# megapose6d/megapose6d

Hardware: NVIDIA H100
Metric: pose hypotheses/sec through render+coarse+5x refine (higher is better)
Workload: dtype f16

## Files before the change

megapose6d_b200/csrc/conv_wgmma.cu:

```cuda
#include <cuda.h>
#include <vector>
#include "mpx_common.cuh"

namespace mpx {

#ifdef MPX_ACT_BF16
#define kTmaActType CU_TENSOR_MAP_DATA_TYPE_BFLOAT16
#define MPX_WGMMA_AB "bf16.bf16"
#else
#define kTmaActType CU_TENSOR_MAP_DATA_TYPE_FLOAT16
#define MPX_WGMMA_AB "f16.f16"
#endif

__device__ __forceinline__ void mbar_init(uint64_t* bar, uint32_t count) {
  asm volatile("mbarrier.init.shared::cta.b64 [%0], %1;" ::"r"(smem_u32(bar)), "r"(count));
}
__device__ __forceinline__ void mbar_expect_tx(uint64_t* bar, uint32_t bytes) {
  asm volatile("mbarrier.arrive.expect_tx.shared::cta.b64 _, [%0], %1;" ::"r"(smem_u32(bar)), "r"(bytes) : "memory");
}
__device__ __forceinline__ void mbar_arrive(uint64_t* bar) {
  asm volatile("mbarrier.arrive.shared::cta.b64 _, [%0];" ::"r"(smem_u32(bar)) : "memory");
}
__device__ __forceinline__ bool mbar_try_wait(uint64_t* bar, uint32_t parity) {
  uint32_t ok;
// ... 34 lines not shown
__device__ __forceinline__ void wgmma_commit() { asm volatile("wgmma.commit_group.sync.aligned;" ::: "memory"); }
template <int N>
__device__ __forceinline__ void wgmma_wait() {
  asm volatile("wgmma.wait_group.sync.aligned %0;" ::"n"(N) : "memory");
}

__device__ __forceinline__ void wgmma_m64n64k16(float (&d)[32], uint64_t desc_a, uint64_t desc_b, uint32_t accumulate) {
  asm volatile(
      "{\n\t.reg .pred p;\n\tsetp.ne.b32 p, %34, 0;\n\t"
      "wgmma.mma_async.sync.aligned.m64n64k16.f32." MPX_WGMMA_AB " "
      "{%0, %1, %2, %3, %4, %5, %6, %7, %8, %9, %10, %11, %12, %13, %14, %15, %16, %17, %18, %19, %20, %21, %22, %23, %24, %25, %26, %27, %28, %29, %30, %31}, %32, %33, p, 1, 1, 0, 0;\n\t}"
      : "+f"(d[0]), "+f"(d[1]), "+f"(d[2]), "+f"(d[3]), "+f"(d[4]), "+f"(d[5]), "+f"(d[6]), "+f"(d[7]), "+f"(d[8]), "+f"(d[9]), "+f"(d[10]), "+f"(d[11]), "+f"(d[12]), "+f"(d[13]), "+f"(d[14]), "+f"(d[15]), "+f"(d[16]), "+f"(d[17]), "+f"(d[18]), "+f"(d[19]), "+f"(d[20]), "+f"(d[21]), "+f"(d[22]), "+f"(d[23]), "+f"(d[24]), "+f"(d[25]), "+f"(d[26]), "+f"(d[27]), "+f"(d[28]), "+f"(d[29]), "+f"(d[30]), "+f"(d[31])
      : "l"(desc_a), "l"(desc_b), "r"(accumulate)
      : "memory");
}
__device__ __forceinline__ void wgmma_m64n128k16(float (&d)[64], uint64_t desc_a, uint64_t desc_b, uint32_t accumulate) {
  asm volatile(
      "{\n\t.reg .pred p;\n\tsetp.ne.b32 p, %66, 0;\n\t"
      "wgmma.mma_async.sync.aligned.m64n128k16.f32." MPX_WGMMA_AB " "
      "{%0, %1, %2, %3, %4, %5, %6, %7, %8, %9, %10, %11, %12, %13, %14, %15, %16, %17, %18, %19, %20, %21, %22, %23, %24, %25, %26, %27, %28, %29, %30, %31, %32, %33, %34, %35, %36, %37, %38, %39, %40, %41, %42, %43, %44, %45, %46, %47, %48, %49, %50, %51, %52, %53, %54, %55, %56, %57, %58, %59, %60, %61, %62, %63}, %64, %65, p, 1, 1, 0, 0;\n\t}"
      : "+f"(d[0]), "+f"(d[1]), "+f"(d[2]), "+f"(d[3]), "+f"(d[4]), "+f"(d[5]), "+f"(d[6]), "+f"(d[7]), "+f"(d[8]), "+f"(d[9]), "+f"(d[10]), "+f"(d[11]), "+f"(d[12]), "+f"(d[13]), "+f"(d[14]), "+f"(d[15]), "+f"(d[16]), "+f"(d[17]), "+f"(d[18]), "+f"(d[19]), "+f"(d[20]), "+f"(d[21]), "+f"(d[22]), "+f"(d[23]), "+f"(d[24]), "+f"(d[25]), "+f"(d[26]), "+f"(d[27]), "+f"(d[28]), "+f"(d[29]), "+f"(d[30]), "+f"(d[31]), "+f"(d[32]), "+f"(d[33]), "+f"(d[34]), "+f"(d[35]), "+f"(d[36]), "+f"(d[37]), "+f"(d[38]), "+f"(d[39]), "+f"(d[40]), "+f"(d[41]), "+f"(d[42]), "+f"(d[43]), "+f"(d[44]), "+f"(d[45]), "+f"(d[46]), "+f"(d[47]), "+f"(d[48]), "+f"(d[49]), "+f"(d[50]), "+f"(d[51]), "+f"(d[52]), "+f"(d[53]), "+f"(d[54]), "+f"(d[55]), "+f"(d[56]), "+f"(d[57]), "+f"(d[58]), "+f"(d[59]), "+f"(d[60]), "+f"(d[61]), "+f"(d[62]), "+f"(d[63])
      : "l"(desc_a), "l"(desc_b), "r"(accumulate)
      : "memory");
}
__device__ __forceinline__ void wgmma_m64n256k16(float (&d)[128], uint64_t desc_a, uint64_t desc_b, uint32_t accumulate) {
  asm volatile(
      "{\n\t.reg .pred p;\n\tsetp.ne.b32 p, %130, 0;\n\t"
      "wgmma.mma_async.sync.aligned.m64n256k16.f32." MPX_WGMMA_AB " "
      "{%0, %1, %2, %3, %4, %5, %6, %7, %8, %9, %10, %11, %12, %13, %14, %15, %16, %17, %18, %19, %20, %21, %22, %23, %24, %25, %26, %27, %28, %29, %30, %31, %32, %33, %34, %35, %36, %37, %38, %39, %40, %41, %42, %43, %44, %45, %46, %47, %48, %49, %50, %51, %52, %53, %54, %55, %56, %57, %58, %59, %60, %61, %62, %63, %64, %65, %66, %67, %68, %69, %70, %71, %72, %73, %74, %75, %76, %77, %78, %79, %80, %81, %82, %83, %84, %85, %86, %87, %88, %89, %90, %91, %92, %93, %94, %95, %96, %97, %98, %99, %100, %101, %102, %103, %104, %105, %106, %107, %108, %109, %110, %111, %112, %113, %114, %115, %116, %117, %118, %119, %120, %121, %122, %123, %124, %125, %126, %127}, %128, %129, p, 1, 1, 0, 0;\n\t}"
      : "+f"(d[0]), "+f"(d[1]), "+f"(d[2]), "+f"(d[3]), "+f"(d[4]), "+f"(d[5]), "+f"(d[6]), "+f"(d[7]), "+f"(d[8]), "+f"(d[9]), "+f"(d[10]), "+f"(d[11]), "+f"(d[12]), "+f"(d[13]), "+f"(d[14]), "+f"(d[15]), "+f"(d[16]), "+f"(d[17]), "+f"(d[18]), "+f"(d[19]), "+f"(d[20]), "+f"(d[21]), "+f"(d[22]), "+f"(d[23]), "+f"(d[24]), "+f"(d[25]), "+f"(d[26]), "+f"(d[27]), "+f"(d[28]), "+f"(d[29]), "+f"(d[30]), "+f"(d[31]), "+f"(d[32]), "+f"(d[33]), "+f"(d[34]), "+f"(d[35]), "+f"(d[36]), "+f"(d[37]), "+f"(d[38]), "+f"(d[39]), "+f"(d[40]), "+f"(d[41]), "+f"(d[42]), "+f"(d[43]), "+f"(d[44]), "+f"(d[45]), "+f"(d[46]), "+f"(d[47]), "+f"(d[48]), "+f"(d[49]), "+f"(d[50]), "+f"(d[51]), "+f"(d[52]), "+f"(d[53]), "+f"(d[54]), "+f"(d[55]), "+f"(d[56]), "+f"(d[57]), "+f"(d[58]), "+f"(d[59]), "+f"(d[60]), "+f"(d[61]), "+f"(d[62]), "+f"(d[63]), "+f"(d[64]), "+f"(d[65]), "+f"(d[66]), "+f"(d[67]), "+f"(d[68]), "+f"(d[69]), "+f"(d[70]), "+f"(d[71]), "+f"(d[72]), "+f"(d[73]), "+f"(d[74]), "+f"(d[75]), "+f"(d[76]), "+f"(d[77]), "+f"(d[78]), "+f"(d[79]), "+f"(d[80]), "+f"(d[81]), "+f"(d[82]), "+f"(d[83]), "+f"(d[84]), "+f"(d[85]), "+f"(d[86]), "+f"(d[87]), "+f"(d[88]), "+f"(d[89]), "+f"(d[90]), "+f"(d[91]), "+f"(d[92]), "+f"(d[93]), "+f"(d[94]), "+f"(d[95]), "+f"(d[96]), "+f"(d[97]), "+f"(d[98]), "+f"(d[99]), "+f"(d[100]), "+f"(d[101]), "+f"(d[102]), "+f"(d[103]), "+f"(d[104]), "+f"(d[105]), "+f"(d[106]), "+f"(d[107]), "+f"(d[108]), "+f"(d[109]), "+f"(d[110]), "+f"(d[111]), "+f"(d[112]), "+f"(d[113]), "+f"(d[114]), "+f"(d[115]), "+f"(d[116]), "+f"(d[117]), "+f"(d[118]), "+f"(d[119]), "+f"(d[120]), "+f"(d[121]), "+f"(d[122]), "+f"(d[123]), "+f"(d[124]), "+f"(d[125]), "+f"(d[126]), "+f"(d[127])
      : "l"(desc_a), "l"(desc_b), "r"(accumulate)
      : "memory");
}
template <int BLOCK_N>
__device__ __forceinline__ void wgmma_tile(float (&d)[BLOCK_N / 2], uint64_t da, uint64_t db, uint32_t accumulate) {
  if constexpr (BLOCK_N == 64) wgmma_m64n64k16(d, da, db, accumulate);
  else if constexpr (BLOCK_N == 128) wgmma_m64n128k16(d, da, db, accumulate);
  else wgmma_m64n256k16(d, da, db, accumulate);
}

__device__ __forceinline__ uint64_t make_sw128_desc(uint32_t smem_addr) {
  uint64_t d = 0;
  d |= static_cast<uint64_t>((smem_addr >> 4) & 0x3FFFu);
  d |= static_cast<uint64_t>(1) << 16;
  d |= static_cast<uint64_t>(64) << 32;
  d |= static_cast<uint64_t>(1) << 62;
  return d;
}

__device__ __forceinline__ uint32_t cluster_ctarank() {
  uint32_t r;
  asm volatile("mov.u32 %0, %%cluster_ctarank;" : "=r"(r));
  return r;
}
__device__ __forceinline__ void cluster_sync_all() {
  asm volatile("barrier.cluster.arrive.release.aligned;" ::: "memory");
  asm volatile("barrier.cluster.wait.acquire.aligned;" ::: "memory");
}
__device__ __forceinline__ void consumers_sync() { asm volatile("bar.sync 1, 256;" ::: "memory"); }

__device__ __forceinline__ void red_max_act4(act_t* dst, uint32_t lo, uint32_t hi) {
#ifdef MPX_ACT_BF16
  asm volatile("red.global.max.noftz.v2.bf16x2 [%0], {%1, %2};" ::"l"(dst), "r"(lo), "r"(hi) : "memory");
#else
  asm volatile("red.global.max.noftz.v2.f16x2 [%0], {%1, %2};" ::"l"(dst), "r"(lo), "r"(hi) : "memory");
#endif
}

struct ProfileSlot {
  cudaEvent_t e0, e1;
// ... 302 lines not shown
        const int px0 = x >> 1, px1 = ((x & 1) && ((x + 1) >> 1) < pq2) ? (x + 1) >> 1 : px0;
        for (int py = py0; py <= py1; ++py) {
          for (int px = px0; px <= px1; ++px) {
            act_t* dst = p.out + ((static_cast<size_t>(img) * pp + py) * pq2 + px) * p.C_out + n0 + col;
#pragma unroll
            for (int j = 0; j < BLOCK_N / 8; ++j) red_max_act4(dst + 8 * j, packed[j], nb[j]);
          }
        }
      }
    }
  }

  __syncthreads();
  if (p.splits > 1) {
    cluster_sync_all();
    const int item = blockIdx.x;
    const int tile = item / p.splits;
    const int m_tile = tile / p.n_tiles;
    const int n_tile = tile - m_tile * p.n_tiles;
    const int n0 = n_tile * BLOCK_N;
    splitk_reduce_slice<BLOCK_N>(smem_u32(smem), p.splits, static_cast<int>(cluster_ctarank()),
                                 static_cast<long long>(m_tile) * kBlockM, p.M_total, p.C_out, n0, p.out, p.residual,
                                 bias_s + n0, p.relu, threadIdx.x, blockDim.x);
    cluster_sync_all();
  }
}

constexpr int kC64Pixels = 256;
constexpr int kC64Stages = 4;
constexpr int kC64ActBytes = kC64Pixels * kBlockK * 2;
constexpr int kC64WBytes = 64 * kBlockK * 2;
constexpr int kC64StageBytes = kC64ActBytes + kC64WBytes;
constexpr int kC64StagingBytes = kC64Pixels * 64 * 2;
constexpr int kC64SmemBytes = kC64Stages * kC64StageBytes + 2 * kC64StagingBytes + 1024  +
                              128  + 256 ;
static_assert(kC64SmemBytes <= 227 * 1024, "conv64: shared memory budget");

struct Conv64Params {
  int M_total, P, Q, S, stride, pad_h, pad_w, cblocks, num_k_blocks, m_tiles;
  int relu;
  int has_residual;
  const float* bias;
};

__device__ __forceinline__ void tma_store_2d(const CUtensorMap* map, const void* smem, int c0, int c1) {
  asm volatile("cp.async.bulk.tensor.2d.global.shared::cta.bulk_group [%0, {%2, %3}], [%1];" ::"l"(map),
               "r"(smem_u32(smem)), "r"(c0), "r"(c1)
               : "memory");
}
__device__ __forceinline__ void bulk_commit() { asm volatile("cp.async.bulk.commit_group;" ::: "memory"); }
__device__ __forceinline__ void bulk_wait_read_all() { asm volatile("cp.async.bulk.wait_group.read 0;" ::: "memory"); }
__device__ __forceinline__ void bulk_wait_all() { asm volatile("cp.async.bulk.wait_group 0;" ::: "memory"); }
__device__ __forceinline__ void fence_proxy_async_smem() { asm volatile("fence.proxy.async.shared::cta;" ::: "memory"); }
__device__ __forceinline__ void warpgroup_sync(int cw) { asm volatile("bar.sync %0, 128;" ::"r"(2 + cw) : "memory"); }
__device__ __forceinline__ void mainloop_turn_wait(int cw) { asm volatile("bar.sync %0, 256;" ::"r"(4 + cw) : "memory"); }
__device__ __forceinline__ void mainloop_turn_pass(int cw) { asm volatile("bar.arrive %0, 256;" ::"r"(5 - cw) : "memory"); }

__host__ __device__ __forceinline__ uint32_t stem_live_steps(int kb, int cblocks, int S) {
  const int tap = kb / cblocks, cb = kb - tap * cblocks;
  const int r = tap / S, s = tap - r * S;
  uint32_t live = 0;
  for (int k = 0; k < 4; ++k) {
    const int slice = (4 * cb + k) / cblocks;
    const int ky = 2 * r + (slice >> 1) - 1, kx = 2 * s + (slice & 1) - 1;
    if (ky >= 0 && ky <= 6 && kx >= 0 && kx <= 6) live |= 1u << k;
  }
  return live;
}

__device__ __forceinline__ void wgmma_kblock(uint32_t live, float (&acc)[128], uint64_t da, uint64_t db) {
  wgmma_fence();
#pragma unroll
  for (int k = 0; k < kBlockK / 16; ++k)
    if (live & (1u << k)) wgmma_m64n256k16(acc, da + static_cast<uint64_t>(2 * k), db + static_cast<uint64_t>(2 * k), 1u);
  wgmma_commit();
}

template <int kStemCblocks>
__global__ void __launch_bounds__(kThreads, 1)
conv64_wgmma_kernel(const __grid_constant__ CUtensorMap map_x, const __grid_constant__ CUtensorMap map_w,
                    const __grid_constant__ CUtensorMap map_res, const __grid_constant__ CUtensorMap map_out,
                    const Conv64Params p) {
  extern __shared__ uint8_t smem_raw[];
  uint8_t* smem = reinterpret_cast<uint8_t*>((reinterpret_cast<uintptr_t>(smem_raw) + 1023) &
                                             ~static_cast<uintptr_t>(1023));
  uint8_t* smem_x = smem;
  uint8_t* smem_w = smem + kC64Stages * kC64ActBytes;
  uint8_t* staging = smem + kC64Stages * kC64StageBytes;
  uint64_t* bars = reinterpret_cast<uint64_t*>(staging + 2 * kC64StagingBytes);
  uint64_t* full_bar = bars;
  uint64_t* empty_bar = bars + kC64Stages;
  uint64_t* res_bar = bars + 2 * kC64Stages;
  float* bias_s = reinterpret_cast<float*>(bars + 16);

  const int wg = __shfl_sync(0xffffffffu, threadIdx.x >> 7, 0);
  const int nk = p.num_k_blocks;
  for (int i = threadIdx.x; i < 64; i += blockDim.x) bias_s[i] = p.bias[i];
  if (threadIdx.x == 0) {
    asm volatile("prefetch.tensormap [%0];" ::"l"(&map_x) : "memory");
    asm volatile("prefetch.tensormap [%0];" ::"l"(&map_w) : "memory");
    asm volatile("prefetch.tensormap [%0];" ::"l"(&map_out) : "memory");
    if (p.has_residual) asm volatile("prefetch.tensormap [%0];" ::"l"(&map_res) : "memory");
    for (int i = 0; i < kC64Stages; ++i) {
      mbar_init(&full_bar[i], 1);
      mbar_init(&empty_bar[i], 4);
    }
    mbar_init(&res_bar[0], 1);
    mbar_init(&res_bar[1], 1);
    asm volatile("fence.mbarrier_init.release.cluster;" ::: "memory");
  }
  pdl_trigger();
  __syncthreads();
  pdl_wait();

  if (wg == 0) {
    asm volatile("setmaxnreg.dec.sync.aligned.u32 40;");
    if (threadIdx.x == 0) {
      int stage = 0;
      uint32_t phase = 0;
      const int pq = p.P * p.Q;
      for (int tile = blockIdx.x; tile < p.m_tiles; tile += gridDim.x) {
        int base_w[2], base_h[2], img[2];
        const int m0 = tile * kC64Pixels;
        const bool second = m0 + kBlockM < p.M_total;
#pragma unroll
        for (int hh = 0; hh < 2; ++hh) {
          const int m = m0 + hh * kBlockM;
          img[hh] = m / pq;
          const int rem = m - img[hh] * pq;
          const int p0 = rem / p.Q;
          base_w[hh] = (rem - p0 * p.Q) * p.stride - p.pad_w;
          base_h[hh] = p0 * p.stride - p.pad_h;
        }
        const uint32_t bytes = (second ? kC64ActBytes : kC64ActBytes / 2) + kC64WBytes;
        int tap = 0, cb = 0;
        for (int kb = 0; kb < nk; ++kb) {
          mbar_wait(&empty_bar[stage], phase ^ 1u);
          mbar_expect_tx(&full_bar[stage], bytes);
          const int r = tap / p.S;
          const int s = tap - r * p.S;
          uint8_t* dst = smem_x + stage * kC64ActBytes;
          tma_load_im2col_4d(dst, &map_x, &full_bar[stage], cb * kBlockK, base_w[0], base_h[0], img[0],
                             static_cast<uint16_t>(s), static_cast<uint16_t>(r));
          if (second)
            tma_load_im2col_4d(dst + kATileBytes, &map_x, &full_bar[stage], cb * kBlockK, base_w[1], base_h[1], img[1],
                               static_cast<uint16_t>(s), static_cast<uint16_t>(r));
          tma_load_2d(smem_w + stage * kC64WBytes, &map_w, &full_bar[stage], kb * kBlockK, 0);
          if (++cb == p.cblocks) {
            cb = 0;
            ++tap;
          }
          if (++stage == kC64Stages) {
            stage = 0;
            phase ^= 1u;
          }
        }
      }
    }
  } else {
    asm volatile("setmaxnreg.inc.sync.aligned.u32 232;");
    const int cw = wg - 1;
    const int t = threadIdx.x & 127;
    const int lane = threadIdx.x & 31;
    const int q = lane >> 2;
    const int c = 16 * (t >> 5) + (q & ~1);
    const int px = 2 * (lane & 3) + (q & 1);
    const bool odd = (q & 1) != 0;
    uint8_t* stage_buf = staging + cw * kC64StagingBytes;
    int local = 0;
    for (int i = cw, tile = blockIdx.x + cw * gridDim.x; tile < p.m_tiles; i += 2, tile += 2 * gridDim.x, ++local) {
      const int m0 = tile * kC64Pixels;
      if (p.has_residual && t == 0) {
        bulk_wait_read_all();
        mbar_expect_tx(&res_bar[cw], kC64StagingBytes);
        tma_load_2d(stage_buf, &map_res, &res_bar[cw], 0, m0);
      }
      const uint32_t g = static_cast<uint32_t>(i) * static_cast<uint32_t>(nk);
      int stage = static_cast<int>(g % kC64Stages);
      uint32_t phase = (g / kC64Stages) & 1u;
      float acc[128];
#pragma unroll
      for (int j = 0; j < 128; ++j) acc[j] = 0.f;
      if (i > 0) mainloop_turn_wait(cw);
      int prev_stage = -1;
      auto kblock = [&](uint32_t live) {
        mbar_wait(&full_bar[stage], phase);
        wgmma_kblock(live, acc, make_sw128_desc(smem_u32(smem_w + stage * kC64WBytes)),
                     make_sw128_desc(smem_u32(smem_x + stage * kC64ActBytes)));
        wgmma_wait<1>();
        if (prev_stage >= 0) {
          __syncwarp();
          if (lane == 0) mbar_arrive(&empty_bar[prev_stage]);
        }
        prev_stage = stage;
        if (++stage == kC64Stages) {
          stage = 0;
          phase ^= 1u;
        }
      };
      if constexpr (kStemCblocks > 0) {
#pragma unroll
        for (int kb = 0; kb < 16 * kStemCblocks; ++kb) kblock(stem_live_steps(kb, kStemCblocks, 4));
      } else {
#pragma unroll 1
        for (int kb = 0; kb < nk; ++kb) kblock(0xFu);
      }
      if (tile + static_cast<int>(gridDim.x) < p.m_tiles) mainloop_turn_pass(cw);
      wgmma_wait<0>();
      __syncwarp();
      if (lane == 0) mbar_arrive(&empty_bar[prev_stage]);

      if (t == 0) bulk_wait_read_all();
      warpgroup_sync(cw);
      if (p.has_residual) mbar_wait(&res_bar[cw], static_cast<uint32_t>(local) & 1u);
      const uint32_t sbase = smem_u32(stage_buf);
#pragma unroll
      for (int h = 0; h < 2; ++h) {
        const float2 b = *reinterpret_cast<const float2*>(bias_s + c + 8 * h);
        const int chunk = (c + 8 * h) >> 3;
#pragma unroll
        for (int j = 0; j < 32; ++j) {
          const float v0 = acc[4 * j + 2 * h], v1 = acc[4 * j + 2 * h + 1];
          const float other = __shfl_xor_sync(0xffffffffu, odd ? v0 : v1, 4);
          float f0 = (odd ? other : v0) + b.x;
          float f1 = (odd ? v1 : other) + b.y;
          const int row = 8 * j + px;
          const uint32_t addr =
              sbase + static_cast<uint32_t>(row * 128 + ((chunk ^ px) << 4) + ((c & 7) << 1));
          if (p.has_residual) {
            uint32_t rr;
            asm volatile("ld.shared.b32 %0, [%1];" : "=r"(rr) : "r"(addr) : "memory");
            const float2 r = unpack_act2(rr);
            f0 += r.x;
            f1 += r.y;
          }
          if (p.relu) {
            f0 = fmaxf(f0, 0.f);
            f1 = fmaxf(f1, 0.f);
          }
          asm volatile("st.shared.b32 [%0], %1;" ::"r"(addr), "r"(pack_act2(f0, f1)) : "memory");
        }
      }
      fence_proxy_async_smem();
      warpgroup_sync(cw);
      if (t == 0) {
        tma_store_2d(&map_out, stage_buf, 0, m0);
        bulk_commit();
      }
    }
    if (t == 0) bulk_wait_all();
  }
}

typedef CUresult (*PFN_encodeTiled)(CUtensorMap*, CUtensorMapDataType, cuuint32_t, void*,
                                    const cuuint64_t*, const cuuint64_t*, const cuuint32_t*,
                                    const cuuint32_t*, CUtensorMapInterleave, CUtensorMapSwizzle,
                                    CUtensorMapL2promotion, CUtensorMapFloatOOBfill);
typedef CUresult (*PFN_encodeIm2col)(CUtensorMap*, CUtensorMapDataType, cuuint32_t, void*,
                                     const cuuint64_t*, const cuuint64_t*, const int*, const int*,
                                     cuuint32_t, cuuint32_t, const cuuint32_t*, CUtensorMapInterleave,
                                     CUtensorMapSwizzle, CUtensorMapL2promotion,
                                     CUtensorMapFloatOOBfill);

static PFN_encodeTiled g_encode_tiled = nullptr;
static PFN_encodeIm2col g_encode_im2col = nullptr;

static int load_driver_entry_points() {
  if (g_encode_tiled && g_encode_im2col) return MPX_OK;
  cudaDriverEntryPointQueryResult q;
  void* f = nullptr;
  MPX_CHECK_CUDA(cudaGetDriverEntryPoint("cuTensorMapEncodeTiled", &f, cudaEnableDefault, &q));
  MPX_REQUIRE(f != nullptr && q == cudaDriverEntryPointSuccess,
              "cuTensorMapEncodeTiled not available from the driver");
  g_encode_tiled = reinterpret_cast<PFN_encodeTiled>(f);
  f = nullptr;
  MPX_CHECK_CUDA(cudaGetDriverEntryPoint("cuTensorMapEncodeIm2col", &f, cudaEnableDefault, &q));
  MPX_REQUIRE(f != nullptr && q == cudaDriverEntryPointSuccess,
              "cuTensorMapEncodeIm2col not available from the driver");
  g_encode_im2col = reinterpret_cast<PFN_encodeIm2col>(f);
// ... 33 lines not shown
                           static_cast<cuuint64_t>(d.W) * d.C_in * 2,
                           static_cast<cuuint64_t>(d.H) * d.W * d.C_in * 2};
  int lower[2] = {-d.pad_lo_w, -d.pad_lo_h};
  int upper[2] = {d.pad_hi_w - (d.S - 1), d.pad_hi_h - (d.R - 1)};
  cuuint32_t estr[4] = {1, static_cast<cuuint32_t>(d.stride), static_cast<cuuint32_t>(d.stride), 1};
  CUresult r = g_encode_im2col(map, kTmaActType, 4, const_cast<void*>(x),
                               dims, strides, lower, upper, kBlockK,
                               kBlockM, estr, CU_TENSOR_MAP_INTERLEAVE_NONE,
                               CU_TENSOR_MAP_SWIZZLE_128B, CU_TENSOR_MAP_L2_PROMOTION_L2_128B,
                               CU_TENSOR_MAP_FLOAT_OOB_FILL_NONE);
  MPX_REQUIRE(r == CUDA_SUCCESS, "cuTensorMapEncodeIm2col failed (%d)", static_cast<int>(r));
  int drv = 0;
  cudaDriverGetVersion(&drv);
  const size_t bytes = static_cast<size_t>(d.n_img) * d.H * d.W * d.C_in * 2;
  if (drv <= 13010 && bytes < 131072) {
    reinterpret_cast<uint64_t*>(map)[1] &= ~(1ull << 21);
  }
  return MPX_OK;
}

static int encode_2d_map(CUtensorMap* map, const void* ptr, cuuint64_t cols, cuuint64_t rows, int box_cols, int box_rows,
                         CUtensorMapL2promotion promo) {
  cuuint64_t dims[2] = {cols, rows};
  cuuint64_t strides[1] = {cols * 2};
  cuuint32_t box[2] = {static_cast<cuuint32_t>(box_cols), static_cast<cuuint32_t>(box_rows)};
  cuuint32_t estr[2] = {1, 1};
  CUresult r = g_encode_tiled(map, kTmaActType, 2, const_cast<void*>(ptr), dims, strides, box, estr,
                              CU_TENSOR_MAP_INTERLEAVE_NONE, CU_TENSOR_MAP_SWIZZLE_128B, promo,
                              CU_TENSOR_MAP_FLOAT_OOB_FILL_NONE);
  MPX_REQUIRE(r == CUDA_SUCCESS, "cuTensorMapEncodeTiled failed (%d)", static_cast<int>(r));
  return MPX_OK;
}

static int conv64_forward(const ConvDesc& d, const CUtensorMap& map_x, const void* w, const float* bias,
                          const void* residual, void* out, int M_total, int P, int Q, int cap, cudaStream_t stream) {
  const int K_total = d.R * d.S * d.C_in;
  CUtensorMap map_w, map_res, map_out;
  int rc = encode_2d_map(&map_w, w, K_total, 64, kBlockK, 64, CU_TENSOR_MAP_L2_PROMOTION_L2_256B);
  if (rc != MPX_OK) return rc;
  rc = encode_2d_map(&map_out, out, 64, M_total, 64, kC64Pixels, CU_TENSOR_MAP_L2_PROMOTION_L2_128B);
  if (rc != MPX_OK) return rc;
  map_res = map_out;
  if (residual != nullptr) {
    rc = encode_2d_map(&map_res, residual, 64, M_total, 64, kC64Pixels, CU_TENSOR_MAP_L2_PROMOTION_L2_128B);
    if (rc != MPX_OK) return rc;
  }
  Conv64Params p{};
  p.M_total = M_total;
  p.P = P;
  p.Q = Q;
  p.S = d.S;
  p.stride = d.stride;
  p.pad_h = d.pad_lo_h;
  p.pad_w = d.pad_lo_w;
  p.cblocks = d.C_in / kBlockK;
  p.num_k_blocks = d.R * d.S * p.cblocks;
  p.m_tiles = (M_total + kC64Pixels - 1) / kC64Pixels;
  p.relu = d.relu;
  p.has_residual = residual != nullptr;
  p.bias = bias;
  const int stem_cblocks = (d.s2d_stem && d.R == 4 && d.S == 4 && p.cblocks <= 2) ? p.cblocks : 0;
  long long live_steps = 0;
  for (int kb = 0; kb < p.num_k_blocks; ++kb)
    live_steps += __builtin_popcount(stem_cblocks ? stem_live_steps(kb, p.cblocks, p.S) : 0xFu);

  static bool attr_set = false;
  if (!attr_set) {
    MPX_CHECK_CUDA(cudaFuncSetAttribute(conv64_wgmma_kernel<0>, cudaFuncAttributeMaxDynamicSharedMemorySize,
                                        kC64SmemBytes));
    MPX_CHECK_CUDA(cudaFuncSetAttribute(conv64_wgmma_kernel<1>, cudaFuncAttributeMaxDynamicSharedMemorySize,
                                        kC64SmemBytes));
    MPX_CHECK_CUDA(cudaFuncSetAttribute(conv64_wgmma_kernel<2>, cudaFuncAttributeMaxDynamicSharedMemorySize,
                                        kC64SmemBytes));
    attr_set = true;
  }
  const int grid = p.m_tiles < cap ? p.m_tiles : cap;
  ProfileSlot* slot = profile_begin(stream);
  void (*kernel)(CUtensorMap, CUtensorMap, CUtensorMap, CUtensorMap, Conv64Params) =
      stem_cblocks == 1 ? conv64_wgmma_kernel<1> : (stem_cblocks == 2 ? conv64_wgmma_kernel<2> : conv64_wgmma_kernel<0>);
  MPX_CHECK_CUDA(launch_pdl(kernel, dim3(grid), dim3(kThreads), kC64SmemBytes, stream, 1, map_x, map_w, map_res, map_out,
                            p));
  MPX_CHECK_CUDA(cudaGetLastError());
  ++g_launches;
  profile_end(slot, stream, 2.0 * M_total * 64 * live_steps * 16);
  return MPX_OK;
}

int conv_forward(const ConvDesc& d, const void* x, const void* w, const float* bias,
                 const void* residual, void* out, int block_n_override, int max_ctas,
                 cudaStream_t stream, int splitk) {
  MPX_REQUIRE(d.C_in % 64 == 0 && d.C_in >= 64, "conv: C_in=%d must be a multiple of 64", d.C_in);
  MPX_REQUIRE(d.C_out % 64 == 0 && d.C_out <= 512, "conv: C_out=%d must be a multiple of 64, at most 512", d.C_out);
  MPX_REQUIRE(d.stride == 1 || d.stride == 2, "conv: stride %d unsupported", d.stride);
  MPX_REQUIRE(d.R >= 1 && d.R <= 8 && d.S >= 1 && d.S <= 8, "conv: filter %dx%d unsupported", d.R, d.S);
  if (d.pool && (!d.relu || residual != nullptr || block_n_override != 0 || splitk != 0)) return MPX_ERR_UNSUPPORTED;
  int rc = load_driver_entry_points();
  if (rc != MPX_OK) return rc;

  const int P = conv_out_dim(d.H, d.pad_lo_h, d.pad_hi_h, d.R, d.stride);
  const int Q = conv_out_dim(d.W, d.pad_lo_w, d.pad_hi_w, d.S, d.stride);
  MPX_REQUIRE(P > 0 && Q > 0, "conv: empty output");
  const long long M_total = static_cast<long long>(d.n_img) * P * Q;
  MPX_REQUIRE(M_total > 0 && M_total < (1LL << 31), "conv: M=%lld out of range", M_total);

  int block_n = block_n_override;
  if (block_n <= 0) {
    const long long m_tiles_est = (M_total + kBlockM - 1) / kBlockM;
    block_n = d.C_out % 256 == 0 ? 256 : (d.C_out % 128 == 0 ? 128 : 64);
    while (block_n > 64 && m_tiles_est * (d.C_out / block_n) < 32) block_n /= 2;
  }
  MPX_REQUIRE((block_n == 64 || block_n == 128 || block_n == 256) && d.C_out % block_n == 0,
              "conv: BLOCK_N=%d invalid for C_out=%d", block_n, d.C_out);

  CUtensorMap map_a, map_b;
  rc = encode_im2col_map(&map_a, d, x);
  if (rc != MPX_OK) return rc;

  const bool aligned = (reinterpret_cast<uintptr_t>(out) & 15) == 0 && (reinterpret_cast<uintptr_t>(residual) & 15) == 0;
  const long long tiles256 = (M_total + kC64Pixels - 1) / kC64Pixels;
  const int cap = max_ctas > 0 ? max_ctas : sm_count();
  if (d.C_out == 64 && block_n_override == 0 && splitk <= 0 && !d.pool && aligned && (g_conv_mode & 4194304) == 0 &&
      ((g_conv_mode & 67108864) != 0 || tiles256 >= 2LL * cap)) {
    const long long m_tiles128 = (M_total + kBlockM - 1) / kBlockM;
    const int nkb = d.R * d.S * (d.C_in / kBlockK);
    if (!(splitk < 0 && m_tiles128 * 2 <= cap && nkb >= 8))
      return conv64_forward(d, map_a, w, bias, residual, out, static_cast<int>(M_total), P, Q, cap, stream);
  }

  rc = encode_2d_map(&map_b, w, static_cast<cuuint64_t>(d.R) * d.S * d.C_in, d.C_out, kBlockK, block_n,
                     CU_TENSOR_MAP_L2_PROMOTION_L2_256B);
  if (rc != MPX_OK) return rc;

  ConvParams p{};
  p.M_total = static_cast<int>(M_total);
  p.P = P;
  p.Q = Q;
  p.C_out = d.C_out;
  p.S = d.S;
  p.stride = d.stride;
  p.pad_h = d.pad_lo_h;
  p.pad_w = d.pad_lo_w;
  p.cblocks = d.C_in / kBlockK;
  p.num_k_blocks = d.R * d.S * p.cblocks;
  p.m_tiles = static_cast<int>((M_total + kBlockM - 1) / kBlockM);
  p.n_tiles = d.C_out / block_n;
  p.relu = d.relu;
  p.pool = d.pool;
  p.bias = bias;
  p.residual = reinterpret_cast<const act_t*>(residual);
  p.out = reinterpret_cast<act_t*>(out);
  p.splits = 1;
  if (splitk != 0) {
    const int tiles = p.m_tiles * p.n_tiles;
    const int sms = max_ctas > 0 ? max_ctas : sm_count();
    int want = splitk > 0 ? splitk : 1;
    if (splitk < 0 && tiles * 2 <= sms && p.num_k_blocks >= 8) {
      want = p.num_k_blocks / 4;
      if (want > sms / tiles) want = sms / tiles;
    }
    const int cap = (splitk < 0 && (g_conv_mode & 524288)) ? 1 : ((splitk < 0 && (g_conv_mode & 262144)) ? 2 : 8);
    int splits = 1;
// ... 16 lines not shown
```

Before: 21560.

## Add row-band producer with resident weights to C_out=64 conv kernel

For stride-1 convs whose padded width fits in a 256-pixel tile, the conv64 kernel now loads a band of input rows once per (row tap, channel block) with a plain 4D tiled TMA. It reuses that band across the S horizontal taps by offsetting the smem descriptor, instead of issuing one im2col load per tap. When they fit, all weights are kept resident in shared memory for the whole kernel. An N=160 wgmma variant handles narrower bands. This cuts redundant activation traffic and weight reloads, at the cost of wasted MMA columns on padded pixels and a more complex barrier scheme.

```diff
diff --git a/megapose6d_b200/csrc/conv_wgmma.cu b/megapose6d_b200/csrc/conv_wgmma.cu
--- a/megapose6d_b200/csrc/conv_wgmma.cu
+++ b/megapose6d_b200/csrc/conv_wgmma.cu
@@ -90,10 +90,20 @@
       : "l"(desc_a), "l"(desc_b), "r"(accumulate)
       : "memory");
 }
+__device__ __forceinline__ void wgmma_m64n160k16(float (&d)[80], uint64_t desc_a, uint64_t desc_b, uint32_t accumulate) {
+  asm volatile(
+      "{\n\t.reg .pred p;\n\tsetp.ne.b32 p, %82, 0;\n\t"
+      "wgmma.mma_async.sync.aligned.m64n160k16.f32." MPX_WGMMA_AB " "
+      "{%0, %1, %2, %3, %4, %5, %6, %7, %8, %9, %10, %11, %12, %13, %14, %15, %16, %17, %18, %19, %20, %21, %22, %23, %24, %25, %26, %27, %28, %29, %30, %31, %32, %33, %34, %35, %36, %37, %38, %39, %40, %41, %42, %43, %44, %45, %46, %47, %48, %49, %50, %51, %52, %53, %54, %55, %56, %57, %58, %59, %60, %61, %62, %63, %64, %65, %66, %67, %68, %69, %70, %71, %72, %73, %74, %75, %76, %77, %78, %79}, %80, %81, p, 1, 1, 0, 0;\n\t}"
+      : "+f"(d[0]), "+f"(d[1]), "+f"(d[2]), "+f"(d[3]), "+f"(d[4]), "+f"(d[5]), "+f"(d[6]), "+f"(d[7]), "+f"(d[8]), "+f"(d[9]), "+f"(d[10]), "+f"(d[11]), "+f"(d[12]), "+f"(d[13]), "+f"(d[14]), "+f"(d[15]), "+f"(d[16]), "+f"(d[17]), "+f"(d[18]), "+f"(d[19]), "+f"(d[20]), "+f"(d[21]), "+f"(d[22]), "+f"(d[23]), "+f"(d[24]), "+f"(d[25]), "+f"(d[26]), "+f"(d[27]), "+f"(d[28]), "+f"(d[29]), "+f"(d[30]), "+f"(d[31]), "+f"(d[32]), "+f"(d[33]), "+f"(d[34]), "+f"(d[35]), "+f"(d[36]), "+f"(d[37]), "+f"(d[38]), "+f"(d[39]), "+f"(d[40]), "+f"(d[41]), "+f"(d[42]), "+f"(d[43]), "+f"(d[44]), "+f"(d[45]), "+f"(d[46]), "+f"(d[47]), "+f"(d[48]), "+f"(d[49]), "+f"(d[50]), "+f"(d[51]), "+f"(d[52]), "+f"(d[53]), "+f"(d[54]), "+f"(d[55]), "+f"(d[56]), "+f"(d[57]), "+f"(d[58]), "+f"(d[59]), "+f"(d[60]), "+f"(d[61]), "+f"(d[62]), "+f"(d[63]), "+f"(d[64]), "+f"(d[65]), "+f"(d[66]), "+f"(d[67]), "+f"(d[68]), "+f"(d[69]), "+f"(d[70]), "+f"(d[71]), "+f"(d[72]), "+f"(d[73]), "+f"(d[74]), "+f"(d[75]), "+f"(d[76]), "+f"(d[77]), "+f"(d[78]), "+f"(d[79])
+      : "l"(desc_a), "l"(desc_b), "r"(accumulate)
+      : "memory");
+}
 template <int BLOCK_N>
 __device__ __forceinline__ void wgmma_tile(float (&d)[BLOCK_N / 2], uint64_t da, uint64_t db, uint32_t accumulate) {
   if constexpr (BLOCK_N == 64) wgmma_m64n64k16(d, da, db, accumulate);
   else if constexpr (BLOCK_N == 128) wgmma_m64n128k16(d, da, db, accumulate);
+  else if constexpr (BLOCK_N == 160) wgmma_m64n160k16(d, da, db, accumulate);
   else wgmma_m64n256k16(d, da, db, accumulate);
 }
 
@@ -462,12 +472,18 @@
 constexpr int kC64WBytes = 64 * kBlockK * 2;
 constexpr int kC64StageBytes = kC64ActBytes + kC64WBytes;
 constexpr int kC64StagingBytes = kC64Pixels * 64 * 2;
-constexpr int kC64SmemBytes = kC64Stages * kC64StageBytes + 2 * kC64StagingBytes + 1024  +
-                              128  + 256 ;
-static_assert(kC64SmemBytes <= 227 * 1024, "conv64: shared memory budget");
+constexpr int kC64BandSlots = 3;
+constexpr int kC64BandWStages = 8;
+static_assert(kC64BandSlots * kC64ActBytes + kC64BandWStages * kC64WBytes == kC64Stages * kC64StageBytes,
+              "conv64: the band producer's ring layout is the im2col producer's");
+constexpr int kC64SmemBytes = 227 * 1024;
+constexpr int kC64BufferBytes = kC64SmemBytes - 1024  - 256  - 256 ;
+static_assert(kC64Stages * kC64StageBytes + 2 * kC64StagingBytes <= kC64BufferBytes, "conv64: shared memory budget");
 
 struct Conv64Params {
   int M_total, P, Q, S, stride, pad_h, pad_w, cblocks, num_k_blocks, m_tiles;
+  int band_w, band_rows, tiles_per_img;
+  int band_slots, slot_bytes, w_resident, w_off, staging_off, staging_bytes;
   int relu;
   int has_residual;
   const float* bias;
@@ -476,6 +492,19 @@
 __device__ __forceinline__ void tma_store_2d(const CUtensorMap* map, const void* smem, int c0, int c1) {
   asm volatile("cp.async.bulk.tensor.2d.global.shared::cta.bulk_group [%0, {%2, %3}], [%1];" ::"l"(map),
                "r"(smem_u32(smem)), "r"(c0), "r"(c1)
+               : "memory");
+}
+__device__ __forceinline__ void tma_load_4d(void* smem, const CUtensorMap* map, uint64_t* bar, int c0, int c1, int c2,
+                                            int c3) {
+  asm volatile(
+      "cp.async.bulk.tensor.4d.shared::cluster.global.tile.mbarrier::complete_tx::bytes"
+      " [%0], [%1, {%3, %4, %5, %6}], [%2];" ::"r"(smem_u32(smem)),
+      "l"(map), "r"(smem_u32(bar)), "r"(c0), "r"(c1), "r"(c2), "r"(c3)
+      : "memory");
+}
+__device__ __forceinline__ void tma_store_4d(const CUtensorMap* map, const void* smem, int c0, int c1, int c2, int c3) {
+  asm volatile("cp.async.bulk.tensor.4d.global.shared::cta.bulk_group [%0, {%2, %3, %4, %5}], [%1];" ::"l"(map),
+               "r"(smem_u32(smem)), "r"(c0), "r"(c1), "r"(c2), "r"(c3)
                : "memory");
 }
 __device__ __forceinline__ void bulk_commit() { asm volatile("cp.async.bulk.commit_group;" ::: "memory"); }
@@ -498,30 +527,40 @@
   return live;
 }
 
-__device__ __forceinline__ void wgmma_kblock(uint32_t live, float (&acc)[128], uint64_t da, uint64_t db) {
+template <int N>
+__device__ __forceinline__ void wgmma_kblock(uint32_t live, float (&acc)[N / 2], uint64_t da, uint64_t db) {
   wgmma_fence();
 #pragma unroll
   for (int k = 0; k < kBlockK / 16; ++k)
-    if (live & (1u << k)) wgmma_m64n256k16(acc, da + static_cast<uint64_t>(2 * k), db + static_cast<uint64_t>(2 * k), 1u);
+    if (live & (1u << k)) wgmma_tile<N>(acc, da + static_cast<uint64_t>(2 * k), db + static_cast<uint64_t>(2 * k), 1u);
   wgmma_commit();
 }
 
-template <int kStemCblocks>
+template <int kStemCblocks, int kBandN>
 __global__ void __launch_bounds__(kThreads, 1)
 conv64_wgmma_kernel(const __grid_constant__ CUtensorMap map_x, const __grid_constant__ CUtensorMap map_w,
                     const __grid_constant__ CUtensorMap map_res, const __grid_constant__ CUtensorMap map_out,
                     const Conv64Params p) {
+  constexpr bool kBand = kBandN > 0;
+  constexpr int kN = kBand ? kBandN : kC64Pixels;
+  constexpr int kStages = kBand ? kC64BandWStages : kC64Stages;
   extern __shared__ uint8_t smem_raw[];
   uint8_t* smem = reinterpret_cast<uint8_t*>((reinterpret_cast<uintptr_t>(smem_raw) + 1023) &
                                              ~static_cast<uintptr_t>(1023));
   uint8_t* smem_x = smem;
-  uint8_t* smem_w = smem + kC64Stages * kC64ActBytes;
-  uint8_t* staging = smem + kC64Stages * kC64StageBytes;
-  uint64_t* bars = reinterpret_cast<uint64_t*>(staging + 2 * kC64StagingBytes);
+  uint8_t* smem_w = smem + (kBand ? p.w_off : kC64Stages * kC64ActBytes);
+  uint8_t* staging = smem + (kBand ? p.staging_off : kC64Stages * kC64StageBytes);
+  const int staging_bytes = kBand ? p.staging_bytes : kC64StagingBytes;
+  const int slot_bytes = kBand ? p.slot_bytes : kC64ActBytes;
+  const bool w_resident = kBand && p.w_resident;
+  uint64_t* bars = reinterpret_cast<uint64_t*>(smem + kC64BufferBytes);
   uint64_t* full_bar = bars;
-  uint64_t* empty_bar = bars + kC64Stages;
-  uint64_t* res_bar = bars + 2 * kC64Stages;
-  float* bias_s = reinterpret_cast<float*>(bars + 16);
+  uint64_t* empty_bar = bars + 8;
+  uint64_t* res_bar = bars + 16;
+  uint64_t* band_full = bars + 18;
+  uint64_t* band_empty = bars + 21;
+  uint64_t* w_bar = bars + 24;
+  float* bias_s = reinterpret_cast<float*>(bars + 32);
 
   const int wg = __shfl_sync(0xffffffffu, threadIdx.x >> 7, 0);
   const int nk = p.num_k_blocks;
@@ -531,9 +570,16 @@
     asm volatile("prefetch.tensormap [%0];" ::"l"(&map_w) : "memory");
     asm volatile("prefetch.tensormap [%0];" ::"l"(&map_out) : "memory");
     if (p.has_residual) asm volatile("prefetch.tensormap [%0];" ::"l"(&map_res) : "memory");
-    for (int i = 0; i < kC64Stages; ++i) {
+    for (int i = 0; i < kStages; ++i) {
       mbar_init(&full_bar[i], 1);
       mbar_init(&empty_bar[i], 4);
+    }
+    if constexpr (kBand) {
+      for (int i = 0; i < kC64BandSlots; ++i) {
+        mbar_init(&band_full[i], 1);
+        mbar_init(&band_empty[i], 4);
+      }
+      mbar_init(w_bar, 1);
     }
     mbar_init(&res_bar[0], 1);
     mbar_init(&res_bar[1], 1);
@@ -548,41 +594,85 @@
     if (threadIdx.x == 0) {
       int stage = 0;
       uint32_t phase = 0;
-      const int pq = p.P * p.Q;
-      for (int tile = blockIdx.x; tile < p.m_tiles; tile += gridDim.x) {
-        int base_w[2], base_h[2], img[2];
-        const int m0 = tile * kC64Pixels;
-        const bool second = m0 + kBlockM < p.M_total;
-#pragma unroll
-        for (int hh = 0; hh < 2; ++hh) {
-          const int m = m0 + hh * kBlockM;
-          img[hh] = m / pq;
-          const int rem = m - img[hh] * pq;
-          const int p0 = rem / p.Q;
-          base_w[hh] = (rem - p0 * p.Q) * p.stride - p.pad_w;
-          base_h[hh] = p0 * p.stride - p.pad_h;
-        }
-        const uint32_t bytes = (second ? kC64ActBytes : kC64ActBytes / 2) + kC64WBytes;
-        int tap = 0, cb = 0;
-        for (int kb = 0; kb < nk; ++kb) {
-          mbar_wait(&empty_bar[stage], phase ^ 1u);
-          mbar_expect_tx(&full_bar[stage], bytes);
-          const int r = tap / p.S;
-          const int s = tap - r * p.S;
-          uint8_t* dst = smem_x + stage * kC64ActBytes;
-          tma_load_im2col_4d(dst, &map_x, &full_bar[stage], cb * kBlockK, base_w[0], base_h[0], img[0],
-                             static_cast<uint16_t>(s), static_cast<uint16_t>(r));
-          if (second)
-            tma_load_im2col_4d(dst + kATileBytes, &map_x, &full_bar[stage], cb * kBlockK, base_w[1], base_h[1], img[1],
+      if constexpr (kBand) {
+        int slot = 0;
+        uint32_t slot_phase = 0;
+        const uint32_t band_bytes = static_cast<uint32_t>(p.band_w * p.band_rows) * 128u;
+        if (w_resident) {
+          mbar_expect_tx(w_bar, static_cast<uint32_t>(nk) * kC64WBytes);
+          for (int kb = 0; kb < nk; ++kb)
+            tma_load_2d(smem_w + kb * kC64WBytes, &map_w, w_bar, kb * kBlockK, 0);
+        }
+        for (int tile = blockIdx.x; tile < p.m_tiles; tile += gridDim.x) {
+          const int img = tile / p.tiles_per_img;
+          const int p0 = (tile - img * p.tiles_per_img) * p.band_rows;
+          int r = 0, s = 0, cb = 0;
+          for (int kb = 0; kb < nk; ++kb) {
+            if (s == 0) {
+              mbar_wait(&band_empty[slot], slot_phase ^ 1u);
+              mbar_expect_tx(&band_full[slot], band_bytes);
+              tma_load_4d(smem_x + slot * slot_bytes, &map_x, &band_full[slot], cb * kBlockK, -p.pad_w,
+                          p0 + r - p.pad_h, img);
+              if (++slot == p.band_slots) {
+                slot = 0;
+                slot_phase ^= 1u;
+              }
+            }
+            if (!w_resident) {
+              mbar_wait(&empty_bar[stage], phase ^ 1u);
+              mbar_expect_tx(&full_bar[stage], kC64WBytes);
+              tma_load_2d(smem_w + stage * kC64WBytes, &map_w, &full_bar[stage], kb * kBlockK, 0);
+              if (++stage == kStages) {
+                stage = 0;
+                phase ^= 1u;
+              }
+            }
+            if (++cb == p.cblocks) {
+              cb = 0;
+              if (++s == p.S) {
+                s = 0;
+                ++r;
+              }
+            }
+          }
+        }
+      } else {
+        const int pq = p.P * p.Q;
+        for (int tile = blockIdx.x; tile < p.m_tiles; tile += gridDim.x) {
+          int base_w[2], base_h[2], img[2];
+          const int m0 = tile * kC64Pixels;
+          const bool second = m0 + kBlockM < p.M_total;
+#pragma unroll
+          for (int hh = 0; hh < 2; ++hh) {
+            const int m = m0 + hh * kBlockM;
+            img[hh] = m / pq;
+            const int rem = m - img[hh] * pq;
+            const int p0 = rem / p.Q;
+            base_w[hh] = (rem - p0 * p.Q) * p.stride - p.pad_w;
+            base_h[hh] = p0 * p.stride - p.pad_h;
+          }
+          const uint32_t bytes = (second ? kC64ActBytes : kC64ActBytes / 2) + kC64WBytes;
+          int tap = 0, cb = 0;
+          for (int kb = 0; kb < nk; ++kb) {
+            mbar_wait(&empty_bar[stage], phase ^ 1u);
+            mbar_expect_tx(&full_bar[stage], bytes);
+            const int r = tap / p.S;
+            const int s = tap - r * p.S;
+            uint8_t* dst = smem_x + stage * kC64ActBytes;
+            tma_load_im2col_4d(dst, &map_x, &full_bar[stage], cb * kBlockK, base_w[0], base_h[0], img[0],
                                static_cast<uint16_t>(s), static_cast<uint16_t>(r));
-          tma_load_2d(smem_w + stage * kC64WBytes, &map_w, &full_bar[stage], kb * kBlockK, 0);
-          if (++cb == p.cblocks) {
-            cb = 0;
-            ++tap;
-          }
-          if (++stage == kC64Stages) {
-            stage = 0;
-            phase ^= 1u;
+            if (second)
+              tma_load_im2col_4d(dst + kATileBytes, &map_x, &full_bar[stage], cb * kBlockK, base_w[1], base_h[1], img[1],
+                                 static_cast<uint16_t>(s), static_cast<uint16_t>(r));
+            tma_load_2d(smem_w + stage * kC64WBytes, &map_w, &full_bar[stage], kb * kBlockK, 0);
+            if (++cb == p.cblocks) {
+              cb = 0;
+              ++tap;
+            }
+            if (++stage == kStages) {
+              stage = 0;
+              phase ^= 1u;
+            }
           }
         }
       }
@@ -596,85 +686,141 @@
     const int c = 16 * (t >> 5) + (q & ~1);
     const int px = 2 * (lane & 3) + (q & 1);
     const bool odd = (q & 1) != 0;
-    uint8_t* stage_buf = staging + cw * kC64StagingBytes;
+    uint8_t* stage_buf = staging + cw * staging_bytes;
+    if (w_resident) mbar_wait(w_bar, 0);
+    const int bands_per_tile = nk / p.S;
     int local = 0;
     for (int i = cw, tile = blockIdx.x + cw * gridDim.x; tile < p.m_tiles; i += 2, tile += 2 * gridDim.x, ++local) {
       const int m0 = tile * kC64Pixels;
+      const int img = kBand ? tile / p.tiles_per_img : 0;
+      const int p0 = kBand ? (tile - img * p.tiles_per_img) * p.band_rows : 0;
       if (p.has_residual && t == 0) {
         bulk_wait_read_all();
-        mbar_expect_tx(&res_bar[cw], kC64StagingBytes);
-        tma_load_2d(stage_buf, &map_res, &res_bar[cw], 0, m0);
+        if constexpr (kBand) {
+          mbar_expect_tx(&res_bar[cw], static_cast<uint32_t>(p.band_rows * p.Q) * 128u);
+          tma_load_4d(stage_buf, &map_res, &res_bar[cw], 0, 0, p0, img);
+        } else {
+          mbar_expect_tx(&res_bar[cw], kC64StagingBytes);
+          tma_load_2d(stage_buf, &map_res, &res_bar[cw], 0, m0);
+        }
       }
       const uint32_t g = static_cast<uint32_t>(i) * static_cast<uint32_t>(nk);
-      int stage = static_cast<int>(g % kC64Stages);
-      uint32_t phase = (g / kC64Stages) & 1u;
-      float acc[128];
-#pragma unroll
-      for (int j = 0; j < 128; ++j) acc[j] = 0.f;
+      int stage = static_cast<int>(g % kStages);
+      uint32_t phase = (g / kStages) & 1u;
+      const uint64_t gb0 = static_cast<uint64_t>(i) * static_cast<uint64_t>(bands_per_tile);
+      const int slot0 = kBand ? static_cast<int>(gb0 % static_cast<uint64_t>(p.band_slots)) : 0;
+      const uint32_t slot_phase0 = kBand ? static_cast<uint32_t>(gb0 / static_cast<uint64_t>(p.band_slots)) & 1u : 0u;
+      float acc[kN / 2];
+#pragma unroll
+      for (int j = 0; j < kN / 2; ++j) acc[j] = 0.f;
       if (i > 0) mainloop_turn_wait(cw);
-      int prev_stage = -1;
-      auto kblock = [&](uint32_t live) {
-        mbar_wait(&full_bar[stage], phase);
-        wgmma_kblock(live, acc, make_sw128_desc(smem_u32(smem_w + stage * kC64WBytes)),
-                     make_sw128_desc(smem_u32(smem_x + stage * kC64ActBytes)));
+      int prev_stage = -1, prev_slot = -1;
+      auto kblock = [&](uint32_t live, int kb, int r, int s, int cb) {
+        uint64_t db;
+        int slot = -1;
+        if constexpr (kBand) {
+          const int u = slot0 + r * p.cblocks + cb;
+          slot = u % p.band_slots;
+          if (s == 0) mbar_wait(&band_full[slot], slot_phase0 ^ (static_cast<uint32_t>(u / p.band_slots) & 1u));
+          db = make_sw128_desc(smem_u32(smem_x + slot * slot_bytes) + static_cast<uint32_t>(s) * 128u);
+        } else {
+          db = make_sw128_desc(smem_u32(smem_x + stage * kC64ActBytes));
+        }
+        uint32_t wa;
+        if (w_resident) {
+          wa = smem_u32(smem_w + kb * kC64WBytes);
+        } else {
+          mbar_wait(&full_bar[stage], phase);
+          wa = smem_u32(smem_w + stage * kC64WBytes);
+        }
+        wgmma_kblock<kN>(live, acc, make_sw128_desc(wa), db);
         wgmma_wait<1>();
-        if (prev_stage >= 0) {
-          __syncwarp();
-          if (lane == 0) mbar_arrive(&empty_bar[prev_stage]);
-        }
-        prev_stage = stage;
-        if (++stage == kC64Stages) {
-          stage = 0;
-          phase ^= 1u;
+        __syncwarp();
+        if (prev_stage >= 0 && lane == 0) mbar_arrive(&empty_bar[prev_stage]);
+        if (prev_slot >= 0 && lane == 0) mbar_arrive(&band_empty[prev_slot]);
+        prev_slot = (kBand && s == p.S - 1) ? slot : -1;
+        if (!w_resident) {
+          prev_stage = stage;
+          if (++stage == kStages) {
+            stage = 0;
+            phase ^= 1u;
+          }
         }
       };
       if constexpr (kStemCblocks > 0) {
 #pragma unroll
-        for (int kb = 0; kb < 16 * kStemCblocks; ++kb) kblock(stem_live_steps(kb, kStemCblocks, 4));
+        for (int kb = 0; kb < 16 * kStemCblocks; ++kb)
+          kblock(stem_live_steps(kb, kStemCblocks, 4), kb, kb / (4 * kStemCblocks), (kb / kStemCblocks) % 4,
+                 kb % kStemCblocks);
       } else {
+        int r = 0, s = 0, cb = 0;
 #pragma unroll 1
-        for (int kb = 0; kb < nk; ++kb) kblock(0xFu);
+        for (int kb = 0; kb < nk; ++kb) {
+          kblock(0xFu, kb, r, s, cb);
+          if (++cb == p.cblocks) {
+            cb = 0;
+            if (++s == p.S) {
+              s = 0;
+              ++r;
+            }
+          }
+        }
       }
       if (tile + static_cast<int>(gridDim.x) < p.m_tiles) mainloop_turn_pass(cw);
       wgmma_wait<0>();
       __syncwarp();
-      if (lane == 0) mbar_arrive(&empty_bar[prev_stage]);
+      if (lane == 0) {
+        if (prev_stage >= 0) mbar_arrive(&empty_bar[prev_stage]);
+        if (prev_slot >= 0) mbar_arrive(&band_empty[prev_slot]);
+      }
 
       if (t == 0) bulk_wait_read_all();
       warpgroup_sync(cw);
       if (p.has_residual) mbar_wait(&res_bar[cw], static_cast<uint32_t>(local) & 1u);
       const uint32_t sbase = smem_u32(stage_buf);
-#pragma unroll
-      for (int h = 0; h < 2; ++h) {
-        const float2 b = *reinterpret_cast<const float2*>(bias_s + c + 8 * h);
-        const int chunk = (c + 8 * h) >> 3;
-#pragma unroll
-        for (int j = 0; j < 32; ++j) {
+      const float2 bias2[2] = {*reinterpret_cast<const float2*>(bias_s + c), *reinterpret_cast<const float2*>(bias_s + c + 8)};
+      const int rows = kBand ? min(p.band_rows, p.P - p0) : 0;
+      int prow = 0, pcol = px;
+#pragma unroll
+      for (int j = 0; j < kN / 8; ++j) {
+        if constexpr (kBand) {
+          while (pcol >= p.band_w) {
+            pcol -= p.band_w;
+            ++prow;
+          }
+        }
+        const bool keep = !kBand || (pcol < p.Q && prow < rows);
+        const int srow = kBand ? prow * p.Q + pcol : 8 * j + px;
+#pragma unroll
+        for (int h = 0; h < 2; ++h) {
           const float v0 = acc[4 * j + 2 * h], v1 = acc[4 * j + 2 * h + 1];
           const float other = __shfl_xor_sync(0xffffffffu, odd ? v0 : v1, 4);
-          float f0 = (odd ? other : v0) + b.x;
-          float f1 = (odd ? v1 : other) + b.y;
-          const int row = 8 * j + px;
-          const uint32_t addr =
-              sbase + static_cast<uint32_t>(row * 128 + ((chunk ^ px) << 4) + ((c & 7) << 1));
-          if (p.has_residual) {
-            uint32_t rr;
-            asm volatile("ld.shared.b32 %0, [%1];" : "=r"(rr) : "r"(addr) : "memory");
-            const float2 r = unpack_act2(rr);
-            f0 += r.x;
-            f1 += r.y;
-          }
-          if (p.relu) {
-            f0 = fmaxf(f0, 0.f);
-            f1 = fmaxf(f1, 0.f);
-          }
-          asm volatile("st.shared.b32 [%0], %1;" ::"r"(addr), "r"(pack_act2(f0, f1)) : "memory");
-        }
+          float f0 = (odd ? other : v0) + bias2[h].x;
+          float f1 = (odd ? v1 : other) + bias2[h].y;
+          const int chunk = (c + 8 * h) >> 3;
+          const uint32_t addr = sbase + static_cast<uint32_t>(srow * 128 + ((chunk ^ (srow & 7)) << 4) + ((c & 7) << 1));
+          if (keep) {
+            if (p.has_residual) {
+              uint32_t rr;
+              asm volatile("ld.shared.b32 %0, [%1];" : "=r"(rr) : "r"(addr) : "memory");
+              const float2 r = unpack_act2(rr);
+              f0 += r.x;
+              f1 += r.y;
+            }
+            if (p.relu) {
+              f0 = fmaxf(f0, 0.f);
+              f1 = fmaxf(f1, 0.f);
+            }
+            asm volatile("st.shared.b32 [%0], %1;" ::"r"(addr), "r"(pack_act2(f0, f1)) : "memory");
+          }
+        }
+        pcol += 8;
       }
       fence_proxy_async_smem();
       warpgroup_sync(cw);
       if (t == 0) {
-        tma_store_2d(&map_out, stage_buf, 0, m0);
+        if constexpr (kBand) tma_store_4d(&map_out, stage_buf, 0, 0, p0, img);
+        else tma_store_2d(&map_out, stage_buf, 0, m0);
         bulk_commit();
       }
     }
@@ -774,19 +920,55 @@
   return MPX_OK;
 }
 
-static int conv64_forward(const ConvDesc& d, const CUtensorMap& map_x, const void* w, const float* bias,
-                          const void* residual, void* out, int M_total, int P, int Q, int cap, cudaStream_t stream) {
+static int encode_nhwc_map(CUtensorMap* map, const void* ptr, int n, int H, int W, int C, int box_w, int box_h) {
+  cuuint64_t dims[4] = {static_cast<cuuint64_t>(C), static_cast<cuuint64_t>(W), static_cast<cuuint64_t>(H),
+                        static_cast<cuuint64_t>(n)};
+  cuuint64_t strides[3] = {static_cast<cuuint64_t>(C) * 2, static_cast<cuuint64_t>(W) * C * 2,
+                           static_cast<cuuint64_t>(H) * W * C * 2};
+  cuuint32_t box[4] = {static_cast<cuuint32_t>(kBlockK), static_cast<cuuint32_t>(box_w), static_cast<cuuint32_t>(box_h),
+                       1};
+  cuuint32_t estr[4] = {1, 1, 1, 1};
+  CUresult r = g_encode_tiled(map, kTmaActType, 4, const_cast<void*>(ptr), dims, strides, box, estr,
+                              CU_TENSOR_MAP_INTERLEAVE_NONE, CU_TENSOR_MAP_SWIZZLE_128B, CU_TENSOR_MAP_L2_PROMOTION_L2_128B,
+                              CU_TENSOR_MAP_FLOAT_OOB_FILL_NONE);
+  MPX_REQUIRE(r == CUDA_SUCCESS, "cuTensorMapEncodeTiled failed (%d)", static_cast<int>(r));
+  return MPX_OK;
+}
+
+static bool conv64_band_fits(const ConvDesc& d) {
+  const int wp = d.W + d.pad_lo_w + d.pad_hi_w;
+  return d.stride == 1 && wp <= kC64Pixels && d.C_in / kBlockK <= kC64BandSlots - 1;
+}
+
+static void conv64_band_layout(Conv64Params& p, int band_n, int S) {
+  auto round1k = [](int b) { return (b + 1023) & ~1023; };
+  const int slot = round1k(p.band_w * p.band_rows * 128);
+  const int staging = round1k(p.band_rows * p.Q * 128);
+  const int weights = p.num_k_blocks * kC64WBytes;
+  const int reach = (band_n + S - 2) * 128 + 128;
+  for (int slots = kC64BandSlots; slots >= p.cblocks + 1; --slots) {
+    const int end = slots * slot + weights + 2 * staging;
+    if (end <= kC64BufferBytes && (slots - 1) * slot + reach <= kC64BufferBytes) {
+      p.band_slots = slots;
+      p.slot_bytes = slot;
+      p.w_resident = 1;
+      p.w_off = slots * slot;
+      p.staging_off = p.w_off + weights;
+      p.staging_bytes = staging;
+      return;
+    }
+  }
+  p.band_slots = kC64BandSlots;
+  p.slot_bytes = kC64ActBytes;
+  p.w_resident = 0;
+  p.w_off = kC64BandSlots * kC64ActBytes;
+  p.staging_off = p.w_off + kC64BandWStages * kC64WBytes;
+  p.staging_bytes = kC64StagingBytes;
+}
+
+static int conv64_forward(const ConvDesc& d, const void* x, const void* w, const float* bias, const void* residual,
+                          void* out, int M_total, int P, int Q, int cap, cudaStream_t stream) {
   const int K_total = d.R * d.S * d.C_in;
-  CUtensorMap map_w, map_res, map_out;
-  int rc = encode_2d_map(&map_w, w, K_total, 64, kBlockK, 64, CU_TENSOR_MAP_L2_PROMOTION_L2_256B);
-  if (rc != MPX_OK) return rc;
-  rc = encode_2d_map(&map_out, out, 64, M_total, 64, kC64Pixels, CU_TENSOR_MAP_L2_PROMOTION_L2_128B);
-  if (rc != MPX_OK) return rc;
-  map_res = map_out;
-  if (residual != nullptr) {
-    rc = encode_2d_map(&map_res, residual, 64, M_total, 64, kC64Pixels, CU_TENSOR_MAP_L2_PROMOTION_L2_128B);
-    if (rc != MPX_OK) return rc;
-  }
   Conv64Params p{};
   p.M_total = M_total;
   p.P = P;
@@ -797,29 +979,63 @@
   p.pad_w = d.pad_lo_w;
   p.cblocks = d.C_in / kBlockK;
   p.num_k_blocks = d.R * d.S * p.cblocks;
-  p.m_tiles = (M_total + kC64Pixels - 1) / kC64Pixels;
   p.relu = d.relu;
   p.has_residual = residual != nullptr;
   p.bias = bias;
+  const bool band = conv64_band_fits(d) && (g_conv_mode & 8388608) == 0;
+  int band_n = 0;
+  CUtensorMap map_x, map_w, map_res, map_out;
+  int rc;
+  if (band) {
+    p.band_w = d.W + d.pad_lo_w + d.pad_hi_w;
+    p.band_rows = kC64Pixels / p.band_w < P ? kC64Pixels / p.band_w : P;
+    p.tiles_per_img = (P + p.band_rows - 1) / p.band_rows;
+    p.m_tiles = d.n_img * p.tiles_per_img;
+    band_n = (p.band_rows - 1) * p.band_w + Q <= 160 ? 160 : 256;
+    conv64_band_layout(p, band_n, d.S);
+    rc = encode_nhwc_map(&map_x, x, d.n_img, d.H, d.W, d.C_in, p.band_w, p.band_rows);
+    if (rc != MPX_OK) return rc;
+    rc = encode_nhwc_map(&map_out, out, d.n_img, P, Q, 64, Q, p.band_rows);
+    if (rc != MPX_OK) return rc;
+    map_res = map_out;
+    if (residual != nullptr) {
+      rc = encode_nhwc_map(&map_res, residual, d.n_img, P, Q, 64, Q, p.band_rows);
+      if (rc != MPX_OK) return rc;
+    }
+  } else {
+    p.m_tiles = (M_total + kC64Pixels - 1) / kC64Pixels;
+    rc = encode_im2col_map(&map_x, d, x);
+    if (rc != MPX_OK) return rc;
+    rc = encode_2d_map(&map_out, out, 64, M_total, 64, kC64Pixels, CU_TENSOR_MAP_L2_PROMOTION_L2_128B);
+    if (rc != MPX_OK) return rc;
+    map_res = map_out;
+    if (residual != nullptr) {
+      rc = encode_2d_map(&map_res, residual, 64, M_total, 64, kC64Pixels, CU_TENSOR_MAP_L2_PROMOTION_L2_128B);
+      if (rc != MPX_OK) return rc;
+    }
+  }
+  rc = encode_2d_map(&map_w, w, K_total, 64, kBlockK, 64, CU_TENSOR_MAP_L2_PROMOTION_L2_256B);
+  if (rc != MPX_OK) return rc;
   const int stem_cblocks = (d.s2d_stem && d.R == 4 && d.S == 4 && p.cblocks <= 2) ? p.cblocks : 0;
   long long live_steps = 0;
   for (int kb = 0; kb < p.num_k_blocks; ++kb)
     live_steps += __builtin_popcount(stem_cblocks ? stem_live_steps(kb, p.cblocks, p.S) : 0xFu);
 
+  typedef void (*Conv64Kernel)(CUtensorMap, CUtensorMap, CUtensorMap, CUtensorMap, Conv64Params);
+  static const Conv64Kernel kernels[3][3] = {
+      {conv64_wgmma_kernel<0, 0>, conv64_wgmma_kernel<0, 160>, conv64_wgmma_kernel<0, 256>},
+      {conv64_wgmma_kernel<1, 0>, conv64_wgmma_kernel<1, 160>, conv64_wgmma_kernel<1, 256>},
+      {conv64_wgmma_kernel<2, 0>, conv64_wgmma_kernel<2, 160>, conv64_wgmma_kernel<2, 256>}};
   static bool attr_set = false;
   if (!attr_set) {
-    MPX_CHECK_CUDA(cudaFuncSetAttribute(conv64_wgmma_kernel<0>, cudaFuncAttributeMaxDynamicSharedMemorySize,
-                                        kC64SmemBytes));
-    MPX_CHECK_CUDA(cudaFuncSetAttribute(conv64_wgmma_kernel<1>, cudaFuncAttributeMaxDynamicSharedMemorySize,
-                                        kC64SmemBytes));
-    MPX_CHECK_CUDA(cudaFuncSetAttribute(conv64_wgmma_kernel<2>, cudaFuncAttributeMaxDynamicSharedMemorySize,
-                                        kC64SmemBytes));
+    for (int a = 0; a < 3; ++a)
+      for (int b = 0; b < 3; ++b)
+        MPX_CHECK_CUDA(cudaFuncSetAttribute(kernels[a][b], cudaFuncAttributeMaxDynamicSharedMemorySize, kC64SmemBytes));
     attr_set = true;
   }
   const int grid = p.m_tiles < cap ? p.m_tiles : cap;
   ProfileSlot* slot = profile_begin(stream);
-  void (*kernel)(CUtensorMap, CUtensorMap, CUtensorMap, CUtensorMap, Conv64Params) =
-      stem_cblocks == 1 ? conv64_wgmma_kernel<1> : (stem_cblocks == 2 ? conv64_wgmma_kernel<2> : conv64_wgmma_kernel<0>);
+  const Conv64Kernel kernel = kernels[stem_cblocks][band_n == 0 ? 0 : (band_n == 160 ? 1 : 2)];
   MPX_CHECK_CUDA(launch_pdl(kernel, dim3(grid), dim3(kThreads), kC64SmemBytes, stream, 1, map_x, map_w, map_res, map_out,
                             p));
   MPX_CHECK_CUDA(cudaGetLastError());
@@ -854,10 +1070,6 @@
   MPX_REQUIRE((block_n == 64 || block_n == 128 || block_n == 256) && d.C_out % block_n == 0,
               "conv: BLOCK_N=%d invalid for C_out=%d", block_n, d.C_out);
 
-  CUtensorMap map_a, map_b;
-  rc = encode_im2col_map(&map_a, d, x);
-  if (rc != MPX_OK) return rc;
-
   const bool aligned = (reinterpret_cast<uintptr_t>(out) & 15) == 0 && (reinterpret_cast<uintptr_t>(residual) & 15) == 0;
   const long long tiles256 = (M_total + kC64Pixels - 1) / kC64Pixels;
   const int cap = max_ctas > 0 ? max_ctas : sm_count();
@@ -866,9 +1078,12 @@
     const long long m_tiles128 = (M_total + kBlockM - 1) / kBlockM;
     const int nkb = d.R * d.S * (d.C_in / kBlockK);
     if (!(splitk < 0 && m_tiles128 * 2 <= cap && nkb >= 8))
-      return conv64_forward(d, map_a, w, bias, residual, out, static_cast<int>(M_total), P, Q, cap, stream);
-  }
-
+      return conv64_forward(d, x, w, bias, residual, out, static_cast<int>(M_total), P, Q, cap, stream);
+  }
+
+  CUtensorMap map_a, map_b;
+  rc = encode_im2col_map(&map_a, d, x);
+  if (rc != MPX_OK) return rc;
   rc = encode_2d_map(&map_b, w, static_cast<cuuint64_t>(d.R) * d.S * d.C_in, d.C_out, kBlockK, block_n,
                      CU_TENSOR_MAP_L2_PROMOTION_L2_256B);
   if (rc != MPX_OK) return rc;
```

Result: faster. 22560, median of 6 (+4.6%).
